# conor722/rust-ray-tracer

Hardware: AMD Instinct MI355X
Metric: Mrays/s (primary) at 1920x1080, Utah teapot (model2.obj) (higher is better)
Workload: dtype f64; 1 GPU; model2.obj 1920x1080, 4 sub-samples/pixel, shadow rays + depth-5 mirror reflection, f64; rays_primary_per_frame=8286720, partition=single launch, octree_nodes=3265, triangles=6334, filter_variant=bundle

## Files before the change

include/rrt.h:

```cpp
#ifndef RRT_H
#define RRT_H
#include <stddef.h>
#include <stdint.h>

#ifdef __cplusplus
extern "C" {
#endif

typedef enum {
    RRT_OK = 0,
    RRT_ERR_INVALID_ARG = -1,
    RRT_ERR_HIP = -2,
    RRT_ERR_OOM = -3,
    RRT_ERR_IO = -4,
    RRT_ERR_PARSE = -5,
    RRT_ERR_DEPTH = -6,
    RRT_ERR_NO_DEVICE = -7,
    RRT_ERR_UNSUPPORTED = -8
} rrt_status;

#define RRT_MAX_OCTREE_DEPTH 40

typedef struct { double x, y, z; } rrt_vec3;

typedef struct { uint32_t kind; uint32_t _pad; double intensity; rrt_vec3 v; } rrt_light;

typedef struct { rrt_vec3 ka, kd, ks; double ns, kr; int32_t tex, bump; } rrt_material;

typedef struct { const uint8_t *rgb; uint32_t width, height; } rrt_texture;

#define RRT_FLAG_NO_CULL 1u
#define RRT_FLAG_LANE_FILTER 2u
#define RRT_FLAG_BUNDLE_FILTER 4u
#define RRT_FLAG_RAY_WALK 8u
#define RRT_FLAG_HOST_SETUP 16u
#define RRT_FLAG_NO_CHAIN_SHORTCUT (1u << 5)

typedef struct {
    double surface_offset;
    uint32_t max_reflection_depth;
    uint32_t flags;
    double vp_w, vp_h, vp_d;
} rrt_options;

typedef struct {
    uint32_t n_tris, n_tris_in_tree;
    uint32_t n_nodes, max_depth;
    uint32_t n_mats, n_tex;
    uint32_t root_own_count, max_own_count;
} rrt_model_info;

// ... 27 lines not shown
void rrt_free(void *p);

typedef struct rrt_raytracer rrt_raytracer;

int rrt_raytracer_create(const rrt_model *m, const rrt_light *lights, uint32_t n_lights, rrt_vec3 origin,
                         const rrt_options *opt, int device, rrt_raytracer **out);
int rrt_raytracer_create_from_arrays(uint32_t n_tris, const double *pos, const double *uv, const double *nrm, const uint32_t *mat,
                                     uint32_t n_mats, const rrt_material *mats, uint32_t n_tex, const rrt_texture *tex, const double *root,
                                     const rrt_light *lights, uint32_t n_lights, rrt_vec3 origin, const rrt_options *opt, int device,
                                     rrt_raytracer **out);
void rrt_raytracer_destroy(rrt_raytracer *rt);

typedef struct { rrt_vec3 eye, right, up, forward; } rrt_camera;
int rrt_raytracer_set_camera(rrt_raytracer *rt, const rrt_camera *cam);
int rrt_raytracer_get_camera(const rrt_raytracer *rt, rrt_camera *out);
int rrt_camera_look_at(rrt_vec3 eye, rrt_vec3 target, rrt_vec3 up_hint, rrt_camera *out);

int rrt_raytracer_set_lights(rrt_raytracer *rt, const rrt_light *lights, uint32_t n_lights);
int rrt_raytracer_get_lights(const rrt_raytracer *rt, rrt_light *out, uint32_t capacity, uint32_t *n_lights);
int rrt_raytracer_set_triangles(rrt_raytracer *rt, uint32_t n_tris, const double *pos, const double *uv, const double *nrm,
                                const uint32_t *mat, const double *root);
int rrt_raytracer_set_triangles_device(rrt_raytracer *rt, uint32_t n_tris, const double *d_pos, const double *d_uv, const double *d_nrm,
                                       const uint32_t *d_mat, const double *root, void *stream);
int rrt_raytracer_release_update_memory(rrt_raytracer *rt);

int rrt_render(rrt_raytracer *rt, uint32_t width, uint32_t height, uint32_t *out_fb);

int rrt_host_buffer_register(void *ptr, size_t bytes);
int rrt_host_buffer_unregister(void *ptr);

// ... 67 lines not shown
```

rust-ray-tracer_amd/__init__.py:

```python
from __future__ import annotations

import ctypes as C
import os
from dataclasses import dataclass
from typing import Iterable, Optional, Sequence

import numpy as np

_HERE = os.path.dirname(os.path.abspath(__file__))
LIB_PATH = os.environ.get("RRT_LIB") or os.path.join(_HERE, "librrt_hip.so")


class RrtError(RuntimeError):
    def __init__(self, status: int, what: str, detail: str):
        super().__init__(f"{what}: {detail or '?'} (status {status})")
        self.status = status
        self.detail = detail


FLAG_NO_CULL, FLAG_LANE_FILTER, FLAG_BUNDLE_FILTER, FLAG_RAY_WALK, FLAG_HOST_SETUP, FLAG_NO_CHAIN_SHORTCUT = 1, 2, 4, 8, 16, 32
BUFFERS = ("nodes", "geom", "attr", "supers", "cboxes", "child_boxes", "tboxes", "suspects", "oct_box", "oct_first_child", "oct_tri_count", "oct_own_off",
           "oct_own_idx", "slot_tri", "slot_pos", "chains")
VARIANT_NAMES = ("lane", "bundle", "ray")

OK, ERR_INVALID_ARG, ERR_HIP, ERR_OOM, ERR_IO, ERR_PARSE, ERR_DEPTH, ERR_NO_DEVICE, ERR_UNSUPPORTED = 0, -1, -2, -3, -4, -5, -6, -7, -8


class Vec3(C.Structure):
    _fields_ = [("x", C.c_double), ("y", C.c_double), ("z", C.c_double)]


class CLight(C.Structure):
    _fields_ = [("kind", C.c_uint32), ("_pad", C.c_uint32), ("intensity", C.c_double), ("v", Vec3)]


# ... 51 lines not shown
    "rrt_model_from_arrays": (C.c_int, [C.c_uint32, _dp, _dp, _dp, _u32p, C.c_uint32, C.POINTER(CMaterial), C.c_uint32, C.POINTER(CTexture), _dp, C.POINTER(_P)]),
    "rrt_model_destroy": (None, [_P]),
    "rrt_model_get_info": (C.c_int, [_P, C.POINTER(CModelInfo)]),
    "rrt_model_get_triangles": (C.c_int, [_P, _dp, _dp, _dp, _u32p]),
    "rrt_model_get_materials": (C.c_int, [_P, C.POINTER(CMaterial)]),
    "rrt_model_get_texture": (C.c_int, [_P, C.c_uint32, C.POINTER(CTexture)]),
    "rrt_model_get_octree": (C.c_int, [_P, _dp, _u32p, _u32p, _u32p, _u32p]),
    "rrt_decode_image_file": (C.c_int, [C.c_char_p, C.POINTER(_u8p), _u32p, _u32p]),
    "rrt_free": (None, [_P]),
    "rrt_raytracer_create": (C.c_int, [_P, C.POINTER(CLight), C.c_uint32, Vec3, C.POINTER(COptions), C.c_int, C.POINTER(_P)]),
    "rrt_raytracer_create_from_arrays": (C.c_int, [C.c_uint32, _dp, _dp, _dp, _u32p, C.c_uint32, C.POINTER(CMaterial), C.c_uint32, C.POINTER(CTexture), _dp,
                                                  C.POINTER(CLight), C.c_uint32, Vec3, C.POINTER(COptions), C.c_int, C.POINTER(_P)]),
    "rrt_raytracer_destroy": (None, [_P]),
    "rrt_raytracer_set_camera": (C.c_int, [_P, C.POINTER(CCamera)]),
    "rrt_raytracer_get_camera": (C.c_int, [_P, C.POINTER(CCamera)]),
    "rrt_camera_look_at": (C.c_int, [Vec3, Vec3, Vec3, C.POINTER(CCamera)]),
    "rrt_raytracer_set_lights": (C.c_int, [_P, C.POINTER(CLight), C.c_uint32]),
    "rrt_raytracer_get_lights": (C.c_int, [_P, C.POINTER(CLight), C.c_uint32, _u32p]),
    "rrt_raytracer_set_triangles": (C.c_int, [_P, C.c_uint32, _dp, _dp, _dp, _u32p, _dp]),
    "rrt_raytracer_set_triangles_device": (C.c_int, [_P, C.c_uint32, _P, _P, _P, _P, _dp, _P]),
    "rrt_raytracer_release_update_memory": (C.c_int, [_P]),
    "rrt_render": (C.c_int, [_P, C.c_uint32, C.c_uint32, _u32p]),
    "rrt_host_buffer_register": (C.c_int, [_P, C.c_size_t]),
    "rrt_host_buffer_unregister": (C.c_int, [_P]),
    "rrt_render_device": (C.c_int, [_P, C.c_uint32, C.c_uint32, _P, _P]),
    "rrt_render_visibility_device": (C.c_int, [_P, C.c_uint32, C.c_uint32, C.POINTER(CRegion), C.POINTER(CVisibility), _P]),
    "rrt_render_visibility": (C.c_int, [_P, C.c_uint32, C.c_uint32, C.POINTER(CRegion), C.POINTER(CVisibility)]),
    "rrt_pick": (C.c_int, [_P, C.c_uint32, C.c_uint32, C.c_uint32, C.c_uint32, C.POINTER(CPickResult)]),
    "rrt_tiles_per_rank": (C.c_uint32, [C.c_uint32, C.c_uint32, C.c_uint32]),
    "rrt_render_tiles_device": (C.c_int, [_P, C.c_uint32, C.c_uint32, C.c_uint32, C.c_uint32, _P, _P]),
# ... 203 lines not shown


def decode_image_file(path: str) -> np.ndarray:
    p = _u8p(); w = C.c_uint32(); h = C.c_uint32()
    _check(lib().rrt_decode_image_file(os.fsencode(path), C.byref(p), C.byref(w), C.byref(h)), f"decode_image_file({path})")
    try:
        return np.ctypeslib.as_array(p, shape=(h.value, w.value, 3)).copy()
    finally:
        lib().rrt_free(p)


class RayTracer:

    def __init__(self, scene_data: SceneData, lights: Iterable[Light], origin: Vector3d = DEFAULT_ORIGIN, device: int = 0,
                 surface_offset: float = 0.0001, max_reflection_depth: int = 5, viewport=(1.0, 1.0, 1.0), no_cull: bool = False,
                 box_filter: Optional[str] = None, host_setup: bool = False, chain_shortcut: bool = True):
        self.scene_data, self.origin, self.device = scene_data, origin, device
        lights = list(lights)
        cl = (CLight * max(1, len(lights)))()
        for i, l in enumerate(lights):
            cl[i] = CLight(l.kind, 0, float(l.intensity), l.v._c())
        flags = (FLAG_NO_CULL if no_cull else 0) | (FLAG_HOST_SETUP if host_setup else 0) | (0 if chain_shortcut else FLAG_NO_CHAIN_SHORTCUT) | {None: 0, "lane": FLAG_LANE_FILTER, "bundle": FLAG_BUNDLE_FILTER, "ray": FLAG_RAY_WALK}[box_filter]
        opt = COptions(surface_offset, max_reflection_depth, flags, *map(float, viewport))
        out = _P()
        _check(lib().rrt_raytracer_create(scene_data._h, cl, len(lights), origin._c(), C.byref(opt), device, C.byref(out)), "rrt_raytracer_create")
        self._h = out

    @classmethod
    def from_arrays(cls, pos, uv, nrm, mat, materials: Sequence[dict], textures: Sequence[np.ndarray], lights: Iterable[Light], origin: Vector3d = DEFAULT_ORIGIN,
                    device: int = 0, root=DEFAULT_ROOT, no_cull: bool = False, box_filter: Optional[str] = None) -> "RayTracer":
        self = cls.__new__(cls)
        self.scene_data, self.origin, self.device = None, origin, device
        lights = list(lights)
        a = _marshal_arrays(pos, uv, nrm, mat, materials, textures, root)
        cl = (CLight * max(1, len(lights)))()
        for i, l in enumerate(lights):
            cl[i] = CLight(l.kind, 0, float(l.intensity), l.v._c())
# ... 43 lines not shown

    def set_camera(self, eye, right=(1.0, 0.0, 0.0), up=(0.0, 1.0, 0.0), forward=(0.0, 0.0, 1.0)) -> None:
        c = CCamera(_vec3(eye), _vec3(right), _vec3(up), _vec3(forward))
        _check(lib().rrt_raytracer_set_camera(self._h, C.byref(c)), "rrt_raytracer_set_camera")

    def look_at(self, eye, target, up=(0.0, 1.0, 0.0)) -> None:
        self.set_camera(**look_at(eye, target, up))

    def reset_camera(self) -> None:
        _check(lib().rrt_raytracer_set_camera(self._h, None), "rrt_raytracer_set_camera")

    def camera(self) -> dict:
        c = CCamera()
        _check(lib().rrt_raytracer_get_camera(self._h, C.byref(c)), "rrt_raytracer_get_camera")
        return _camera_dict(c)

    def set_lights(self, lights: Iterable[Light]) -> None:
        lights = list(lights)
        cl = (CLight * max(1, len(lights)))()
        for i, l in enumerate(lights):
            cl[i] = CLight(l.kind, 0, float(l.intensity), l.v._c())
        _check(lib().rrt_raytracer_set_lights(self._h, cl, len(lights)), "rrt_raytracer_set_lights")

    def lights(self) -> list:
        n = C.c_uint32(0)
        _check(lib().rrt_raytracer_get_lights(self._h, None, 0, C.byref(n)), "rrt_raytracer_get_lights")
        cl = (CLight * max(1, n.value))()
        _check(lib().rrt_raytracer_get_lights(self._h, cl, n.value, C.byref(n)), "rrt_raytracer_get_lights")
        return [Light(l.kind, l.intensity, Vector3d(l.v.x, l.v.y, l.v.z)) for l in cl[:n.value]]

# ... 315 lines not shown
```

rust-ray-tracer_amd/csrc/api_internal.hpp:

```cpp
#pragma once
#include <cstdint>
#include <new>
#include <string>
#include <vector>

#include "device_memory.hpp"
#include "device_scene.hpp"
#include "hip_check.hpp"
#include "model.hpp"
#include "scene_build.hpp"

struct rrt_model { rrt::Model m; };

struct rrt_raytracer {
    int device = 0;
    rrt::DevScene scene{};
    rrt_options opt{};
    rrt::BuiltScene built;
    rrt::DevBuf table_mem; rrt::DevArena tables;
#ifdef RRT_PROFILE
    rrt::DevBuf prof_mem;
#endif
    uint64_t scene_bytes = 0;
    hipEvent_t ev0 = nullptr, ev1 = nullptr;
    rrt_stats stats{};
    bool stats_pending = false;
    bool launched = false;
    int walk = 0;
    int walk_rays = -1;
    bool variant_forced = false;
    rrt::KeptBuf host_fb;
    rrt::KeptBuf vis_buf;
    rrt::KeptBuf tune_buf;
    uint32_t n_chains = 0, n_chain_nodes = 0;
    double upload_ms = 0, hip_init_ms = 0, create_ms = 0;
    bool gpu_setup = false;
    struct Buf { const void* p = nullptr; size_t bytes = 0; } bufs[16];
    hipStream_t own_stream = nullptr;
    uint32_t tuned_w = 0, tuned_h = 0, tuned_world = 0;
    uint32_t size_frames = 0;
    bool size_measured = false;
    rrt_camera cam{};
    rrt_vec3 origin0{};
    rrt::DevBuf guard_mem;
    rrt::Box root{};
    uint64_t built_bytes = 0;
    rrt::BuildMemory update_mem;
};
// ... 48 lines not shown
```

rust-ray-tracer_amd/csrc/device_scene.hpp:

```cpp
#pragma once
#include <cstdint>

namespace rrt {

struct DevNode {
    double lo[3], hi[3];
    double mid[3];
    uint32_t first_child;
    uint32_t sup_begin;
    uint32_t sup_count;
    uint32_t flags;
    uint32_t s0_begin;
    uint32_t leaf_base;
};
static_assert(sizeof(DevNode) == 96, "DevNode must be 96 bytes");

struct DevTriGeom { double v1[3], e1[3], e2[3]; uint32_t pos, _pad; };
static_assert(sizeof(DevTriGeom) == 80, "DevTriGeom must be 80 bytes");
__host__ __device__ inline double edge_canon(double x) {
    uint64_t b; __builtin_memcpy(&b, &x, 8);
    if ((b & 0x7FF0000000000000ull) == 0x7FF0000000000000ull && (b & 0x000FFFFFFFFFFFFFull) != 0ull) b = 0x7FF8000000000000ull;
    __builtin_memcpy(&x, &b, 8);
    return x;
}
// ... 50 lines not shown
    DevLight lights[RRT_MAX_LIGHTS];
#ifdef RRT_PROFILE
    unsigned long long* prof;
#endif
};

struct FrameParams {
    uint32_t width, height;
    double x_scale, y_scale, z_value;
    uint32_t tiles_x, tiles_y;
    uint32_t rank, world;
    uint32_t tiled_output;
    uint32_t xcd_chunk;
    uint32_t tile_begin, tile_end, row_begin, row_end;
    double right[3], up[3], forward[3];
};

struct VisParams {
    FrameParams F;
    uint32_t col_begin, col_end;
    uint32_t tile_x0, tile_y0, tiles_w, _pad;
    uint8_t* hit; double *t, *u, *v; uint32_t* tri; uint32_t* albedo;
};

int launch_render(const DevScene& s, const FrameParams& f, uint32_t* d_out, void* stream, int walk);
int launch_visibility(const DevScene& s, const VisParams& p, void* stream, int walk);
int launch_detile(uint32_t width, uint32_t height, uint32_t world, const uint32_t* d_gathered, uint32_t* d_fb, void* stream);
int launch_ray_colours(const DevScene& s, uint32_t n, const double* d_origins, const double* d_dirs, uint32_t* d_colours, void* stream, int walk);
int launch_intersect(const DevScene& s, uint32_t n, const double* d_origins, const double* d_dirs, const double* d_max_t,
                     uint8_t* d_hit, double* d_t, double* d_u, double* d_v, uint32_t* d_tri, void* stream, int walk);
int launch_occlusion(const DevScene& s, uint32_t n, const double* d_origins, const double* d_dirs, const double* d_max_t, uint8_t* d_occluded, void* stream, int walk);
struct SuspectRecord { uint32_t tri; uint32_t _pad; DevSuspect s; };
int launch_suspects_resident(const DevTriGeom* geom, const DevTriAttr* attr, uint32_t n_list_slots, const double eye[3], double pad,
                             uint32_t* d_count, SuspectRecord* d_out, void* stream);
uint32_t stack_bytes_per_wave(uint32_t levels);
void preload_kernels();

}
```

rust-ray-tracer_amd/csrc/frames.cpp:

```cpp
#include <algorithm>
#include <cstdlib>
#include <cstring>

#include "api_internal.hpp"
#include "staging.hpp"

namespace {

using namespace rrt;

FrameParams frame_params(const rrt_raytracer* rt, uint32_t width, uint32_t height, uint32_t rank, uint32_t world, bool tiled) {
    FrameParams f{};
    f.width = width; f.height = height;
    f.x_scale = rt->opt.vp_w / (double)width;
    f.y_scale = rt->opt.vp_h / (double)height;
    f.z_value = rt->opt.vp_d;
    f.tiles_x = (width + 7) / 8; f.tiles_y = (height + 7) / 8;
    f.rank = rank; f.world = world; f.tiled_output = tiled ? 1u : 0u;
    f.tile_begin = 0; f.tile_end = f.tiles_x * f.tiles_y; f.row_begin = 0; f.row_end = height;
    const rrt_camera& c = rt->cam;
    f.right[0] = c.right.x; f.right[1] = c.right.y; f.right[2] = c.right.z;
    f.up[0] = c.up.x; f.up[1] = c.up.y; f.up[2] = c.up.z;
    f.forward[0] = c.forward.x; f.forward[1] = c.forward.y; f.forward[2] = c.forward.z;
    static const int forced = [] { const char* e = std::getenv("RRT_XCD_CHUNK"); return e ? std::atoi(e) : -1; }();
// ... 80 lines not shown
    if (rt->variant_forced) return rt->walk;
    if (rt->walk_rays >= 0) return rt->walk_rays;
    if (n < kTuneMinRays) return rt->walk;
    return measure_rays(rt, [&](int variant) { return launch(std::min(n, kTuneSample), variant); });
}
int device_rays_variant(const rrt_raytracer* rt) {
    if (rt->variant_forced) return rt->walk;
    return rt->walk_rays >= 0 ? rt->walk_rays : rt->walk;
}
void check_rays(const rrt_raytracer* rt, uint32_t n, const double* origins, const double* dirs, bool outputs_ok) {
    if (!rt) throw Error{RRT_ERR_INVALID_ARG, "null raytracer"};
    if (n && (!origins || !dirs)) throw Error{RRT_ERR_INVALID_ARG, "null ray origins or directions"};
    if (n && !outputs_ok) throw Error{RRT_ERR_INVALID_ARG, "null output: a device form needs one output pointer at least, a host form every one of its outputs"};
}

void launch_frame(rrt_raytracer* rt, uint32_t width, uint32_t height, uint32_t rank, uint32_t world, bool tiled, void* d_out, void* stream) {
    DeviceGuard guard(rt->device);
    const FrameParams f = frame_params(rt, width, height, rank, world, tiled);
    tune_variant(rt, f, static_cast<uint32_t*>(d_out), stream);
    timed_launch(rt, stream, [&] { return launch_render(rt->scene, f, static_cast<uint32_t*>(d_out), stream, rt->walk); });
    record(rt, width, height, world == 1 ? 4 * traced_pixels(width, height) : 0, rt->walk);
}

int visibility_variant(const rrt_raytracer* rt, uint32_t width, uint32_t height) {
    if (rt->variant_forced) return rt->walk;
    if (rt->tuned_w == width && rt->tuned_h == height && rt->tuned_world == 1u) return rt->walk;
    return first_frame_variant(rt, width, height);
}

constexpr int kPlanes = 6;
constexpr size_t kPlaneElem[kPlanes] = {1, 8, 8, 8, 4, 4};

rrt_region check_visibility(const rrt_raytracer* rt, uint32_t width, uint32_t height, const rrt_region* region, const rrt_visibility* planes) {
// ... 137 lines not shown
        visibility_to_host(rt, width, height, r, *planes);
        return RRT_OK;
    });
}

int rrt_pick(rrt_raytracer* rt, uint32_t width, uint32_t height, uint32_t px, uint32_t py, rrt_pick_result* out) {
    return guarded([&]() -> int {
        check_frame(rt, width, height);
        if (!out) throw Error{RRT_ERR_INVALID_ARG, "null result"};
        if (px >= width || py >= height) throw Error{RRT_ERR_INVALID_ARG, "pixel outside the frame"};
        *out = pick_pixel(rt, width, height, px, py);
        return RRT_OK;
    });
}

int rrt_detile_device(rrt_raytracer* rt, uint32_t width, uint32_t height, uint32_t world, const void* d_gathered, void* d_fb, void* stream) {
    return guarded([&]() -> int {
        check_frame(rt, width, height);
        if (!d_gathered || !d_fb || world == 0) throw Error{RRT_ERR_INVALID_ARG, "bad argument"};
        DeviceGuard guard(rt->device);
        HIP_TRY((hipError_t)launch_detile(width, height, world, static_cast<const uint32_t*>(d_gathered), static_cast<uint32_t*>(d_fb), stream));
        return RRT_OK;
    });
}

int rrt_host_buffer_register(void* ptr, size_t bytes) {
    return guarded([&]() -> int {
        if (!ptr || !bytes) throw Error{RRT_ERR_INVALID_ARG, "null buffer"};
        HIP_TRY(hipHostRegister(ptr, bytes, hipHostRegisterDefault));
        return RRT_OK;
// ... 19 lines not shown
        staged_download(out_fb, d_fb, bytes, rt->own_stream);
        HIP_TRY(hipStreamSynchronize(rt->own_stream));
        return RRT_OK;
    });
}

int rrt_render_progressive(rrt_raytracer* rt, uint32_t width, uint32_t height, uint32_t* out_fb, uint32_t chunk_rows, rrt_update_fn on_update, void* user) {
    return guarded([&]() -> int {
        check_frame(rt, width, height);
        if (!out_fb) throw Error{RRT_ERR_INVALID_ARG, "null framebuffer"};
        if (chunk_rows == 0) chunk_rows = 50;
        DeviceGuard guard(rt->device);
        const size_t bytes = sizeof(uint32_t) * (size_t)width * height;
        uint32_t* d_fb = static_cast<uint32_t*>(rt->host_fb.at_least(bytes));
        FrameParams f = frame_params(rt, width, height, 0, 1, false);
        tune_variant(rt, f, d_fb, nullptr);
        HIP_TRY(hipMemsetAsync(d_fb, 0, bytes, nullptr));
        std::memset(out_fb, 0, bytes);
        const int64_t H = height, half = H / 2;
        timed_launch(rt, nullptr, [&] {
            for (int64_t cs = -half; cs < half; cs += chunk_rows) {
                const int64_t ce = std::min<int64_t>(cs + chunk_rows, half);
                const int64_t r_lo = H - (ce - 1 + half), r_hi = std::min<int64_t>(H - (cs + half), H - 1);
                if (r_lo <= r_hi) {
                    f.row_begin = (uint32_t)r_lo; f.row_end = (uint32_t)r_hi + 1;
                    f.tile_begin = (f.row_begin / 8) * f.tiles_x; f.tile_end = ((f.row_end + 7) / 8) * f.tiles_x;
                    HIP_TRY((hipError_t)launch_render(rt->scene, f, d_fb, nullptr, rt->walk));
                    HIP_TRY(hipMemcpy(out_fb + (size_t)f.row_begin * width, d_fb + (size_t)f.row_begin * width,
                                      sizeof(uint32_t) * (size_t)width * (f.row_end - f.row_begin), hipMemcpyDeviceToHost));
                }
// ... 123 lines not shown
```

rust-ray-tracer_amd/csrc/raytracer.cpp:

```cpp
#include <atomic>
#include <chrono>
#include <cstdio>
#include <cstdlib>
#include <cstring>
#include <functional>
#include <memory>

#include "api_internal.hpp"
#include "parallel.hpp"
#include "staging.hpp"

namespace {

using namespace rrt;

enum { kBufNodes = 0, kBufGeom, kBufAttr, kBufSupers, kBufCboxes, kBufChildBoxes, kBufTboxes, kBufSuspects, kBufOctBox, kBufOctFirstChild, kBufOctTriCount, kBufOctOwnOff, kBufOctOwnIdx, kBufSlotTri, kBufSlotPos, kBufChains, kBufCount };

void alloc_tables(rrt_raytracer* rt, const SceneTables& T) {
    size_t need = (size_t)1 << 16;
    for (auto& t : T.tex) need += (size_t)3 * t.width * t.height + 256;
    need += T.n_mats * sizeof(DevMaterial) + T.tex.size() * sizeof(DevTexture) + 1024;
    rt->table_mem = dev_alloc(need);
    rt->tables.base = static_cast<char*>(rt->table_mem.h); rt->tables.cap = need;
}
// ... 49 lines not shown
        {kBufSlotTri, G.slot_tri, (size_t)G.n_slots_total * 4}, {kBufSlotPos, G.slot_pos, (size_t)G.n_slots_total * 4},
        {kBufChains, G.chains, (size_t)G.n_chains * sizeof(DevChain)}};
    for (const auto& k : kept) { rt->bufs[k.id].p = k.p; rt->bufs[k.id].bytes = k.p ? k.bytes : 0; }
    S.cull_enabled = (o.flags & RRT_FLAG_NO_CULL) ? 0u : 1u;
    S.cull_half_over_limit = S.cull_limit > 0.0f ? 0.5f / S.cull_limit : 0.0f;
    S.inner_shrink = (S.cull_enabled && G.all_inside_root) ? (float)(2.0 * G.pad) : 0.0f;
    rt->n_chains = G.n_chains; rt->n_chain_nodes = G.n_chain_nodes;
    if (!(S.inner_shrink > 0.0f)) { rt->n_chains = 0; rt->n_chain_nodes = 0; }
    S.chains = (rt->n_chains && !(o.flags & RRT_FLAG_NO_CHAIN_SHORTCUT)) ? G.chains : nullptr;
    S.n_suspects = G.n_suspects;
    S.stack_levels = G.max_depth > 1 ? G.max_depth - 1 : 1;
    const uint64_t bytes = (uint64_t)G.n_nodes * sizeof(DevNode) + (uint64_t)G.n_slots_total * (sizeof(DevTriGeom) + sizeof(DevTriAttr))
                         + ((uint64_t)G.n_sup_records + n_cboxes + n_child_boxes + n_tboxes) * 32;
    rt->scene_bytes += bytes - rt->built_bytes;
    rt->built_bytes = bytes;
}

void check_lights(const rrt_light* lights, uint32_t n_lights) {
    if (n_lights && !lights) throw Error{RRT_ERR_INVALID_ARG, "null light list"};
    if (n_lights > RRT_MAX_LIGHTS) throw Error{RRT_ERR_INVALID_ARG, "too many lights (max 16)"};
    for (uint32_t i = 0; i < n_lights; i++) if (lights[i].kind > 2) throw Error{RRT_ERR_INVALID_ARG, "bad light kind"};
}

void store_lights(rrt_raytracer* rt, const rrt_light* lights, uint32_t n_lights) {
    DevScene& S = rt->scene;
    S.n_lights = n_lights;
    for (uint32_t i = 0; i < n_lights; i++) {
        S.lights[i].kind = lights[i].kind; S.lights[i]._pad = 0; S.lights[i].intensity = lights[i].intensity;
        S.lights[i].v[0] = lights[i].v.x; S.lights[i].v[1] = lights[i].v.y; S.lights[i].v[2] = lights[i].v.z;
    }
// ... 208 lines not shown
```

rust-ray-tracer_amd/csrc/render.hip:

```cpp
#include <hip/hip_runtime.h>

#include <cmath>
#include <type_traits>

#include "device_scene.hpp"

#ifndef RRT_TU
#define RRT_TU 0
#endif
#define RRT_TU_FRAME (RRT_TU == 0 || RRT_TU == 1)
#define RRT_TU_LANE (RRT_TU == 0 || RRT_TU == 3)
#define RRT_TU_RAYS (RRT_TU == 0 || RRT_TU == 2)

namespace rrt {
namespace {

#define RRT_CONSTANT __attribute__((address_space(4)))
constexpr double kEps = 2.220446049250313e-16;
constexpr uint32_t kNone = 0xFFFFFFFFu;
constexpr double kInf = __builtin_huge_val();

struct V3 { double x, y, z; };
__device__ __forceinline__ V3 mk(double x, double y, double z) { V3 r; r.x = x; r.y = y; r.z = z; return r; }
__device__ __forceinline__ V3 ld3(const double* p) { return mk(p[0], p[1], p[2]); }
// ... 1234 lines not shown
    uint32_t blk = blockIdx.x;
    if (F.xcd_chunk) {
        const uint32_t C = F.xcd_chunk, full = (gridDim.x / (8u * C)) * (8u * C);
        if (blk < full) { const uint32_t xcd = blk & 7u, i = blk >> 3; blk = ((i / C) * 8u + xcd) * C + (i % C); }
    }
    const uint32_t local_tile = blk >> 2, quad = blk & 3u;
    const uint32_t pix = lane >> 2, sub = lane & 3u;
    const uint32_t tile = F.tile_begin + local_tile * F.world + F.rank;
    const bool tile_ok = tile < F.tile_end;
    const uint32_t tx = tile_ok ? tile % F.tiles_x : 0, ty = tile_ok ? tile / F.tiles_x : 0;
    const uint32_t px = tx * 8 + (quad & 1u) * 4 + (pix & 3u);
    const uint32_t py = ty * 8 + (quad >> 1) * 4 + (pix >> 2);
    const int32_t W = (int32_t)F.width, H = (int32_t)F.height;
    const bool in_fb = tile_ok && (int32_t)px < W && py >= F.row_begin && py < F.row_end;
    const bool traced = in_fb && (int32_t)px < 2 * (W / 2) && (int32_t)py >= H - 2 * (H / 2) + 1;
    const int32_t x = (int32_t)px - W / 2;
    const int32_t y = (H - H / 2) - (int32_t)py;
    const double xd = (sub & 1u) ? ((double)x + 0.5) : (double)x;
    const double yd = (sub & 2u) ? ((double)y + 0.5) : (double)y;
    const double sa = xd * F.x_scale, sb = yd * F.y_scale, sc = F.z_value;
    const V3 dir = mk((F.right[0] * sa + F.up[0] * sb) + F.forward[0] * sc,
                      (F.right[1] * sa + F.up[1] * sb) + F.forward[1] * sc,
                      (F.right[2] * sa + F.up[2] * sb) + F.forward[2] * sc);
#ifdef RRT_PROFILE
    Prof prof{}; prof.last = __builtin_amdgcn_s_memtime();
    const unsigned long long wave_rt0 = __builtin_amdgcn_s_memrealtime(); (void)wave_rt0;
#endif
    const uint32_t c = trace_colour<kWalk, kGroups, true>(PROF_ARG S, stk, traced, ld3(S.origin), dir);
#if defined(RRT_PROFILE) && defined(RRT_PROF_WAVETIME)
    {
        constexpr unsigned long long kRealtimeTicksPerUs = 100ull;
        const unsigned long long ticks = __builtin_amdgcn_s_memrealtime() - wave_rt0;
        const uint32_t us = (uint32_t)(ticks / kRealtimeTicksPerUs);
        const uint32_t bucket = us < 2u ? 0u : (uint32_t)(31 - __builtin_clz(us));
        if (lane == 0) { atomicAdd(S.prof + (bucket < 15u ? bucket : 15u), 1ull); atomicMax(S.prof + 16, ticks); }
    }
#elif defined(RRT_PROFILE)
    PROF_T(4);
    for (int i = 0; i < 16; i++) if (prof.c[i]) atomicAdd(S.prof + i, prof.c[i]);
    if (lane == 0) { for (int i = 0; i < 8; i++) if (prof.t[i]) atomicAdd(S.prof + 16 + i, prof.t[i]); }
    for (int i = 0; i < 4; i++) if (prof.b[i]) atomicAdd(S.prof + 24 + i, prof.b[i]);
#endif
    uint32_t r = (c >> 16) & 255u, g = (c >> 8) & 255u, b = c & 255u;
// ... 323 lines not shown
```

rust-ray-tracer_amd/csrc/scene_build.hip:

```cpp
#include <cfloat>
#include <cmath>
#include <cstdio>
#include <cstdlib>
#include <cstring>

#include <hip/hip_runtime.h>
#include <rocprim/rocprim.hpp>

#include <algorithm>
#include <chrono>
#include <memory>
#include <string>
#include <vector>

#include "parallel.hpp"
#include "scene_build.hpp"
#include "staging.hpp"

namespace rrt {
namespace {

constexpr uint32_t kNone = 0xFFFFFFFFu;
constexpr int kBlock = 256;
constexpr uint32_t kClusterTris = 8, kSuperTris = 64, kGroupSupers = 8, kGroupThreshold = 24;
// ... 539 lines not shown
    const double v1[3] = {t.v1.x, t.v1.y, t.v1.z};
    const double e1[3] = {t.v2.x - t.v1.x, t.v2.y - t.v1.y, t.v2.z - t.v1.z}, e2[3] = {t.v3.x - t.v1.x, t.v3.y - t.v1.y, t.v3.z - t.v1.z};
    DevSuspect q;
    if (suspect_of(v1, e1, e2, ox, oy, oz, pad, q)) suspect_append(i, q, count, out);
}
__global__ void __launch_bounds__(kBlock) k_suspects_resident(const DevTriGeom* __restrict__ geom, const DevTriAttr* __restrict__ attr, uint32_t n_list_slots,
                                                              double ox, double oy, double oz, double pad, uint32_t* count, SuspectRecord* out) {
    const uint32_t s = blockIdx.x * kBlock + threadIdx.x;
    if (s >= n_list_slots) return;
    const DevTriGeom& g = geom[s];
    const double v1[3] = {g.v1[0], g.v1[1], g.v1[2]}, e1[3] = {g.e1[0], g.e1[1], g.e1[2]}, e2[3] = {g.e2[0], g.e2[1], g.e2[2]};
    DevSuspect q;
    if (suspect_of(v1, e1, e2, ox, oy, oz, pad, q)) suspect_append(attr[s].orig, q, count, out);
}

__global__ void __launch_bounds__(kBlock) k_pack_triangles(const double* __restrict__ pos, const double* __restrict__ uv, const double* __restrict__ nrm, const uint32_t* __restrict__ mat, uint32_t n, Triangle* __restrict__ out) {
    const uint32_t i = blockIdx.x * kBlock + threadIdx.x;
    if (i >= n) return;
    auto rd = [](const double* p) { Vec3 v; v.x = p[0]; v.y = p[1]; v.z = p[2]; return v; };
    Triangle t;
    t.v1 = rd(pos + 9 * (size_t)i); t.v2 = rd(pos + 9 * (size_t)i + 3); t.v3 = rd(pos + 9 * (size_t)i + 6);
    t.t1 = rd(uv + 9 * (size_t)i);  t.t2 = rd(uv + 9 * (size_t)i + 3);  t.t3 = rd(uv + 9 * (size_t)i + 6);
    t.n1 = rd(nrm + 9 * (size_t)i); t.n2 = rd(nrm + 9 * (size_t)i + 3); t.n3 = rd(nrm + 9 * (size_t)i + 6);
    t.mat = mat[i]; t._pad = 0;
    out[i] = t;
}
__global__ void __launch_bounds__(kBlock) k_count_bad_materials(const uint32_t* __restrict__ mat, uint32_t n, uint32_t n_mats, uint32_t* count) {
    __shared__ uint32_t block_count;
    if (threadIdx.x == 0) block_count = 0u;
    __syncthreads();
// ... 282 lines not shown
    if (e != hipSuccess) return (int)e;
    if (n == 0) return 0;
    hipLaunchKernelGGL(k_count_bad_materials, dim3(std::min(grid_for(n), 1024u)), dim3(kBlock), 0, st, d_mat, n, n_mats, d_count);
    return (int)hipGetLastError();
}

int launch_suspects_resident(const DevTriGeom* geom, const DevTriAttr* attr, uint32_t n_list_slots, const double eye[3], double pad, uint32_t* d_count, SuspectRecord* d_out, void* stream) {
    hipStream_t st = (hipStream_t)stream;
    hipError_t e = hipMemsetAsync(d_count, 0, sizeof(uint32_t), st);
    if (e != hipSuccess) return (int)e;
    if (n_list_slots == 0) return 0;
    hipLaunchKernelGGL(k_suspects_resident, dim3(grid_for(n_list_slots)), dim3(kBlock), 0, st, geom, attr, n_list_slots, eye[0], eye[1], eye[2], pad, d_count, d_out);
    return (int)hipGetLastError();
}

}
```

Baseline: 10450 Mrays/s.

## Skip tracing screen quads that no triangle cluster box can project onto

A new kernel projects every leaf cluster bounding box through the camera with conservative error bounds. It sets bits in a per-resolution mask of 4x4-pixel quads, and any degenerate or unsafe case falls back to a full mask. The render kernel reads this mask and, for uncovered quads, writes the background colour directly without building a ray or walking the hierarchy. The mask is cached per resolution and keyed on camera, viewport and scene epoch, so it is rebuilt only when those change. The cost is an extra small launch whenever the view changes, plus correctness risk if the conservative bounds are ever too tight.

```diff
diff --git a/include/rrt.h b/include/rrt.h
--- a/include/rrt.h
+++ b/include/rrt.h
@@ -35,6 +35,7 @@
 #define RRT_FLAG_RAY_WALK 8u
 #define RRT_FLAG_HOST_SETUP 16u
 #define RRT_FLAG_NO_CHAIN_SHORTCUT (1u << 5)
+#define RRT_FLAG_NO_COVERAGE (1u << 6)
 
 typedef struct {
     double surface_offset;
@@ -92,6 +93,7 @@
 typedef struct { rrt_vec3 eye, right, up, forward; } rrt_camera;
 int rrt_raytracer_set_camera(rrt_raytracer *rt, const rrt_camera *cam);
 int rrt_raytracer_get_camera(const rrt_raytracer *rt, rrt_camera *out);
+int rrt_raytracer_get_coverage(rrt_raytracer *rt, uint32_t width, uint32_t height, uint32_t *words, uint32_t capacity, uint32_t *n_words, uint32_t *flags);
 int rrt_camera_look_at(rrt_vec3 eye, rrt_vec3 target, rrt_vec3 up_hint, rrt_camera *out);
 
 int rrt_raytracer_set_lights(rrt_raytracer *rt, const rrt_light *lights, uint32_t n_lights);
diff --git a/rust-ray-tracer_amd/__init__.py b/rust-ray-tracer_amd/__init__.py
--- a/rust-ray-tracer_amd/__init__.py
+++ b/rust-ray-tracer_amd/__init__.py
@@ -18,7 +18,7 @@
         self.detail = detail
 
 
-FLAG_NO_CULL, FLAG_LANE_FILTER, FLAG_BUNDLE_FILTER, FLAG_RAY_WALK, FLAG_HOST_SETUP, FLAG_NO_CHAIN_SHORTCUT = 1, 2, 4, 8, 16, 32
+FLAG_NO_CULL, FLAG_LANE_FILTER, FLAG_BUNDLE_FILTER, FLAG_RAY_WALK, FLAG_HOST_SETUP, FLAG_NO_CHAIN_SHORTCUT, FLAG_NO_COVERAGE = 1, 2, 4, 8, 16, 32, 64
 BUFFERS = ("nodes", "geom", "attr", "supers", "cboxes", "child_boxes", "tboxes", "suspects", "oct_box", "oct_first_child", "oct_tri_count", "oct_own_off",
            "oct_own_idx", "slot_tri", "slot_pos", "chains")
 VARIANT_NAMES = ("lane", "bundle", "ray")
@@ -100,6 +100,7 @@
     "rrt_raytracer_destroy": (None, [_P]),
     "rrt_raytracer_set_camera": (C.c_int, [_P, C.POINTER(CCamera)]),
     "rrt_raytracer_get_camera": (C.c_int, [_P, C.POINTER(CCamera)]),
+    "rrt_raytracer_get_coverage": (C.c_int, [_P, C.c_uint32, C.c_uint32, _u32p, C.c_uint32, _u32p, _u32p]),
     "rrt_camera_look_at": (C.c_int, [Vec3, Vec3, Vec3, C.POINTER(CCamera)]),
     "rrt_raytracer_set_lights": (C.c_int, [_P, C.POINTER(CLight), C.c_uint32]),
     "rrt_raytracer_get_lights": (C.c_int, [_P, C.POINTER(CLight), C.c_uint32, _u32p]),
@@ -333,13 +334,13 @@
 
     def __init__(self, scene_data: SceneData, lights: Iterable[Light], origin: Vector3d = DEFAULT_ORIGIN, device: int = 0,
                  surface_offset: float = 0.0001, max_reflection_depth: int = 5, viewport=(1.0, 1.0, 1.0), no_cull: bool = False,
-                 box_filter: Optional[str] = None, host_setup: bool = False, chain_shortcut: bool = True):
+                 box_filter: Optional[str] = None, host_setup: bool = False, chain_shortcut: bool = True, coverage: bool = True):
         self.scene_data, self.origin, self.device = scene_data, origin, device
         lights = list(lights)
         cl = (CLight * max(1, len(lights)))()
         for i, l in enumerate(lights):
             cl[i] = CLight(l.kind, 0, float(l.intensity), l.v._c())
-        flags = (FLAG_NO_CULL if no_cull else 0) | (FLAG_HOST_SETUP if host_setup else 0) | (0 if chain_shortcut else FLAG_NO_CHAIN_SHORTCUT) | {None: 0, "lane": FLAG_LANE_FILTER, "bundle": FLAG_BUNDLE_FILTER, "ray": FLAG_RAY_WALK}[box_filter]
+        flags = (FLAG_NO_CULL if no_cull else 0) | (FLAG_HOST_SETUP if host_setup else 0) | (0 if chain_shortcut else FLAG_NO_CHAIN_SHORTCUT) | (0 if coverage else FLAG_NO_COVERAGE) | {None: 0, "lane": FLAG_LANE_FILTER, "bundle": FLAG_BUNDLE_FILTER, "ray": FLAG_RAY_WALK}[box_filter]
         opt = COptions(surface_offset, max_reflection_depth, flags, *map(float, viewport))
         out = _P()
         _check(lib().rrt_raytracer_create(scene_data._h, cl, len(lights), origin._c(), C.byref(opt), device, C.byref(out)), "rrt_raytracer_create")
@@ -413,6 +414,15 @@
         c = CCamera()
         _check(lib().rrt_raytracer_get_camera(self._h, C.byref(c)), "rrt_raytracer_get_camera")
         return _camera_dict(c)
+
+    def coverage(self, w: int, h: int) -> dict:
+        n = C.c_uint32(0); fl = C.c_uint32(0)
+        _check(lib().rrt_raytracer_get_coverage(self._h, w, h, None, 0, C.byref(n), C.byref(fl)), "rrt_raytracer_get_coverage")
+        words = np.full(n.value, 0xFFFFFFFF, np.uint32)
+        _check(lib().rrt_raytracer_get_coverage(self._h, w, h, words.ctypes.data_as(_u32p), n.value, None, C.byref(fl)), "rrt_raytracer_get_coverage")
+        qx, qy = 2 * ((w + 7) // 8), 2 * ((h + 7) // 8)
+        bits = np.unpackbits(words.view(np.uint8), bitorder="little")[:qx * qy].reshape(qy, qx).astype(bool)
+        return {"bits": bits, "in_use": bool(fl.value & 1), "full": bool(fl.value & 2)}
 
     def set_lights(self, lights: Iterable[Light]) -> None:
         lights = list(lights)
diff --git a/rust-ray-tracer_amd/csrc/api_internal.hpp b/rust-ray-tracer_amd/csrc/api_internal.hpp
--- a/rust-ray-tracer_amd/csrc/api_internal.hpp
+++ b/rust-ray-tracer_amd/csrc/api_internal.hpp
@@ -11,6 +11,20 @@
 #include "scene_build.hpp"
 
 struct rrt_model { rrt::Model m; };
+
+namespace rrt {
+struct CoverageMask {
+    uint32_t width = 0, height = 0, n_words = 0;
+    struct Key { uint64_t epoch; double v[15]; } key{};
+    bool valid = false;
+    bool in_use = false;
+    KeptBuf buf;
+    HipOwned<hipEvent_t, hipEventDestroy> built;
+    hipStream_t built_on = nullptr;
+    bool settled = false;
+};
+constexpr size_t kMaxCoverageSizes = 8;
+}
 
 struct rrt_raytracer {
     int device = 0;
@@ -32,6 +46,8 @@
     rrt::KeptBuf host_fb;
     rrt::KeptBuf vis_buf;
     rrt::KeptBuf tune_buf;
+    std::vector<rrt::CoverageMask> coverage;
+    uint64_t scene_epoch = 0;
     uint32_t n_chains = 0, n_chain_nodes = 0;
     double upload_ms = 0, hip_init_ms = 0, create_ms = 0;
     bool gpu_setup = false;
diff --git a/rust-ray-tracer_amd/csrc/device_scene.hpp b/rust-ray-tracer_amd/csrc/device_scene.hpp
--- a/rust-ray-tracer_amd/csrc/device_scene.hpp
+++ b/rust-ray-tracer_amd/csrc/device_scene.hpp
@@ -88,6 +88,7 @@
     uint32_t xcd_chunk;
     uint32_t tile_begin, tile_end, row_begin, row_end;
     double right[3], up[3], forward[3];
+    const uint32_t* coverage;
 };
 
 struct VisParams {
@@ -107,6 +108,13 @@
 struct SuspectRecord { uint32_t tri; uint32_t _pad; DevSuspect s; };
 int launch_suspects_resident(const DevTriGeom* geom, const DevTriAttr* attr, uint32_t n_list_slots, const double eye[3], double pad,
                              uint32_t* d_count, SuspectRecord* d_out, void* stream);
+struct CoverageView {
+    double eye[3];
+    double inv[9];
+    double z_value, x_scale, y_scale;
+    uint32_t width, height, quads_x, quads_y;
+};
+int launch_coverage(const DevClusterBox* tboxes, uint32_t n_list_slots, const CoverageView& v, uint32_t* d_mask, uint32_t n_words, void* stream);
 uint32_t stack_bytes_per_wave(uint32_t levels);
 void preload_kernels();
 
diff --git a/rust-ray-tracer_amd/csrc/frames.cpp b/rust-ray-tracer_amd/csrc/frames.cpp
--- a/rust-ray-tracer_amd/csrc/frames.cpp
+++ b/rust-ray-tracer_amd/csrc/frames.cpp
@@ -1,4 +1,5 @@
 #include <algorithm>
+#include <cmath>
 #include <cstdlib>
 #include <cstring>
 
@@ -118,9 +119,81 @@
     if (n && !outputs_ok) throw Error{RRT_ERR_INVALID_ARG, "null output: a device form needs one output pointer at least, a host form every one of its outputs"};
 }
 
+bool coverage_view(const rrt_raytracer* rt, uint32_t width, uint32_t height, CoverageView& v) {
+    static const bool env_on = [] { const char* e = std::getenv("RRT_COVERAGE"); return !(e && std::atoi(e) == 0); }();
+    const DevScene& S = rt->scene;
+    if (!env_on || (rt->opt.flags & (RRT_FLAG_NO_CULL | RRT_FLAG_NO_COVERAGE)) || !S.cull_enabled || !(rt->built.pad > 0) || S.n_suspects > 0 || S.n_slots >= 50000u) return false;
+    const FrameParams f = frame_params(rt, width, height, 0, 1, false);
+    if (!(f.z_value != 0.0) || !std::isfinite(f.z_value) || !std::isfinite(f.x_scale) || !std::isfinite(f.y_scale)) return false;
+    const double* r = f.right; const double* u = f.up; const double* w = f.forward;
+    const double cof[9] = {u[1] * w[2] - u[2] * w[1], u[2] * w[0] - u[0] * w[2], u[0] * w[1] - u[1] * w[0],
+                           w[1] * r[2] - w[2] * r[1], w[2] * r[0] - w[0] * r[2], w[0] * r[1] - w[1] * r[0],
+                           r[1] * u[2] - r[2] * u[1], r[2] * u[0] - r[0] * u[2], r[0] * u[1] - r[1] * u[0]};
+    const double det = r[0] * cof[0] + r[1] * cof[1] + r[2] * cof[2];
+    if (!(det != 0.0) || !std::isfinite(det)) return false;
+    double norm_m = 0, norm_inv = 0;
+    for (int i = 0; i < 3; i++) {
+        double row = 0;
+        for (int k = 0; k < 3; k++) { v.inv[3 * i + k] = cof[3 * i + k] / det; row += std::fabs(v.inv[3 * i + k]); }
+        norm_inv = std::max(norm_inv, row);
+        norm_m = std::max(norm_m, std::fabs(r[i]) + std::fabs(u[i]) + std::fabs(w[i]));
+    }
+    if (!std::isfinite(norm_inv) || !(norm_m * norm_inv <= 0x1p16)) return false;
+    const double limit = S.cull_limit;
+    if (!std::isfinite(limit)) return false;
+    const double ha = std::fabs(f.x_scale) * (width / 2 + 1.0), hb = std::fabs(f.y_scale) * (height / 2 + 1.0), hc = std::fabs(f.z_value);
+    for (int k = 0; k < 3; k++) {
+        if (!(std::fabs(S.origin[k]) <= limit)) return false;
+        if (!(std::fabs(r[k]) * ha + std::fabs(u[k]) * hb + std::fabs(w[k]) * hc <= limit)) return false;
+        v.eye[k] = S.origin[k];
+    }
+    v.z_value = f.z_value; v.x_scale = f.x_scale; v.y_scale = f.y_scale;
+    v.width = width; v.height = height; v.quads_x = 2 * f.tiles_x; v.quads_y = 2 * f.tiles_y;
+    return true;
+}
+
+CoverageMask* ensure_coverage(rrt_raytracer* rt, uint32_t width, uint32_t height, void* stream) {
+    CoverageMask* m = nullptr;
+    for (CoverageMask& c : rt->coverage) if (c.width == width && c.height == height) m = &c;
+    if (!m) {
+        if (rt->coverage.size() >= kMaxCoverageSizes) return nullptr;
+        rt->coverage.emplace_back();
+        m = &rt->coverage.back(); m->width = width; m->height = height;
+    }
+    CoverageMask::Key key{};
+    key.epoch = rt->scene_epoch;
+    const rrt_camera& c = rt->cam;
+    const double vals[15] = {rt->scene.origin[0], rt->scene.origin[1], rt->scene.origin[2], c.right.x, c.right.y, c.right.z, c.up.x, c.up.y, c.up.z,
+                             c.forward.x, c.forward.y, c.forward.z, rt->opt.vp_w, rt->opt.vp_h, rt->opt.vp_d};
+    std::memcpy(key.v, vals, sizeof vals);
+    if (!(m->valid && std::memcmp(&m->key, &key, sizeof key) == 0)) {
+        m->valid = false;
+        CoverageView v{};
+        m->in_use = coverage_view(rt, width, height, v);
+        if (m->in_use) {
+            m->n_words = (v.quads_x * v.quads_y + 31u) / 32u;
+            uint32_t* d_mask = static_cast<uint32_t*>(m->buf.at_least(sizeof(uint32_t) * ((size_t)m->n_words + 1)));
+            if (!m->built.h) HIP_TRY(hipEventCreateWithFlags(&m->built.h, hipEventDisableTiming));
+            HIP_TRY((hipError_t)launch_coverage(rt->scene.tboxes, rt->built.n_list_slots, v, d_mask, m->n_words, stream));
+            HIP_TRY(hipEventRecord(m->built.h, (hipStream_t)stream));
+            m->built_on = (hipStream_t)stream; m->settled = false;
+        }
+        m->key = key; m->valid = true;
+    } else if (m->in_use && !m->settled) {
+        if (hipEventQuery(m->built.h) == hipSuccess) m->settled = true;
+        else if ((hipStream_t)stream != m->built_on) HIP_TRY(hipStreamWaitEvent((hipStream_t)stream, m->built.h, 0));
+    }
+    return m->in_use ? m : nullptr;
+}
+const uint32_t* coverage_words(rrt_raytracer* rt, uint32_t width, uint32_t height, void* stream) {
+    const CoverageMask* m = ensure_coverage(rt, width, height, stream);
+    return m ? static_cast<const uint32_t*>(m->buf.mem.h) : nullptr;
+}
+
 void launch_frame(rrt_raytracer* rt, uint32_t width, uint32_t height, uint32_t rank, uint32_t world, bool tiled, void* d_out, void* stream) {
     DeviceGuard guard(rt->device);
-    const FrameParams f = frame_params(rt, width, height, rank, world, tiled);
+    FrameParams f = frame_params(rt, width, height, rank, world, tiled);
+    f.coverage = coverage_words(rt, width, height, stream);
     tune_variant(rt, f, static_cast<uint32_t*>(d_out), stream);
     timed_launch(rt, stream, [&] { return launch_render(rt->scene, f, static_cast<uint32_t*>(d_out), stream, rt->walk); });
     record(rt, width, height, world == 1 ? 4 * traced_pixels(width, height) : 0, rt->walk);
@@ -288,6 +361,30 @@
     });
 }
 
+int rrt_raytracer_get_coverage(rrt_raytracer* rt, uint32_t width, uint32_t height, uint32_t* words, uint32_t capacity, uint32_t* n_words, uint32_t* flags) {
+    return guarded([&]() -> int {
+        check_frame(rt, width, height);
+        if (capacity && !words) throw Error{RRT_ERR_INVALID_ARG, "null words with a non-zero capacity"};
+        DeviceGuard guard(rt->device);
+        const uint32_t n = (4u * ((width + 7) / 8) * ((height + 7) / 8) + 31u) / 32u;
+        if (n_words) *n_words = n;
+        if (!rt->own_stream) rt->own_stream = (hipStream_t)setup_stream();
+        const CoverageMask* m = ensure_coverage(rt, width, height, rt->own_stream);
+        uint32_t fl = 0;
+        if (m) {
+            const uint32_t* d_mask = static_cast<const uint32_t*>(m->buf.mem.h);
+            uint32_t full = 0;
+            const uint32_t k = std::min(capacity, m->n_words);
+            if (k) HIP_TRY(hipMemcpyAsync(words, d_mask, sizeof(uint32_t) * (size_t)k, hipMemcpyDeviceToHost, rt->own_stream));
+            HIP_TRY(hipMemcpyAsync(&full, d_mask + m->n_words, sizeof full, hipMemcpyDeviceToHost, rt->own_stream));
+            HIP_TRY(hipStreamSynchronize(rt->own_stream));
+            fl = 1u | (full ? 2u : 0u);
+        }
+        if (flags) *flags = fl;
+        return RRT_OK;
+    });
+}
+
 int rrt_detile_device(rrt_raytracer* rt, uint32_t width, uint32_t height, uint32_t world, const void* d_gathered, void* d_fb, void* stream) {
     return guarded([&]() -> int {
         check_frame(rt, width, height);
@@ -337,6 +434,7 @@
         const size_t bytes = sizeof(uint32_t) * (size_t)width * height;
         uint32_t* d_fb = static_cast<uint32_t*>(rt->host_fb.at_least(bytes));
         FrameParams f = frame_params(rt, width, height, 0, 1, false);
+        f.coverage = coverage_words(rt, width, height, nullptr);
         tune_variant(rt, f, d_fb, nullptr);
         HIP_TRY(hipMemsetAsync(d_fb, 0, bytes, nullptr));
         std::memset(out_fb, 0, bytes);
diff --git a/rust-ray-tracer_amd/csrc/raytracer.cpp b/rust-ray-tracer_amd/csrc/raytracer.cpp
--- a/rust-ray-tracer_amd/csrc/raytracer.cpp
+++ b/rust-ray-tracer_amd/csrc/raytracer.cpp
@@ -87,6 +87,7 @@
                          + ((uint64_t)G.n_sup_records + n_cboxes + n_child_boxes + n_tboxes) * 32;
     rt->scene_bytes += bytes - rt->built_bytes;
     rt->built_bytes = bytes;
+    rt->scene_epoch++;
 }
 
 void check_lights(const rrt_light* lights, uint32_t n_lights) {
diff --git a/rust-ray-tracer_amd/csrc/render.hip b/rust-ray-tracer_amd/csrc/render.hip
--- a/rust-ray-tracer_amd/csrc/render.hip
+++ b/rust-ray-tracer_amd/csrc/render.hip
@@ -1272,19 +1272,27 @@
     const int32_t W = (int32_t)F.width, H = (int32_t)F.height;
     const bool in_fb = tile_ok && (int32_t)px < W && py >= F.row_begin && py < F.row_end;
     const bool traced = in_fb && (int32_t)px < 2 * (W / 2) && (int32_t)py >= H - 2 * (H / 2) + 1;
-    const int32_t x = (int32_t)px - W / 2;
-    const int32_t y = (H - H / 2) - (int32_t)py;
-    const double xd = (sub & 1u) ? ((double)x + 0.5) : (double)x;
-    const double yd = (sub & 2u) ? ((double)y + 0.5) : (double)y;
-    const double sa = xd * F.x_scale, sb = yd * F.y_scale, sc = F.z_value;
-    const V3 dir = mk((F.right[0] * sa + F.up[0] * sb) + F.forward[0] * sc,
-                      (F.right[1] * sa + F.up[1] * sb) + F.forward[1] * sc,
-                      (F.right[2] * sa + F.up[2] * sb) + F.forward[2] * sc);
+    bool covered = true;
+    if (F.coverage) {
+        const uint32_t bit = (2u * ty + (quad >> 1)) * (2u * F.tiles_x) + 2u * tx + (quad & 1u);
+        covered = ((((const RRT_CONSTANT uint32_t*)F.coverage)[bit >> 5] >> (bit & 31u)) & 1u) != 0u;
+    }
 #ifdef RRT_PROFILE
     Prof prof{}; prof.last = __builtin_amdgcn_s_memtime();
     const unsigned long long wave_rt0 = __builtin_amdgcn_s_memrealtime(); (void)wave_rt0;
 #endif
-    const uint32_t c = trace_colour<kWalk, kGroups, true>(PROF_ARG S, stk, traced, ld3(S.origin), dir);
+    uint32_t c = 0x00FFFFFFu;
+    if (covered) {
+        const int32_t x = (int32_t)px - W / 2;
+        const int32_t y = (H - H / 2) - (int32_t)py;
+        const double xd = (sub & 1u) ? ((double)x + 0.5) : (double)x;
+        const double yd = (sub & 2u) ? ((double)y + 0.5) : (double)y;
+        const double sa = xd * F.x_scale, sb = yd * F.y_scale, sc = F.z_value;
+        const V3 dir = mk((F.right[0] * sa + F.up[0] * sb) + F.forward[0] * sc,
+                          (F.right[1] * sa + F.up[1] * sb) + F.forward[1] * sc,
+                          (F.right[2] * sa + F.up[2] * sb) + F.forward[2] * sc);
+        c = trace_colour<kWalk, kGroups, true>(PROF_ARG S, stk, traced, ld3(S.origin), dir);
+    }
 #if defined(RRT_PROFILE) && defined(RRT_PROF_WAVETIME)
     {
         constexpr unsigned long long kRealtimeTicksPerUs = 100ull;
diff --git a/rust-ray-tracer_amd/csrc/scene_build.hip b/rust-ray-tracer_amd/csrc/scene_build.hip
--- a/rust-ray-tracer_amd/csrc/scene_build.hip
+++ b/rust-ray-tracer_amd/csrc/scene_build.hip
@@ -577,6 +577,63 @@
     if (suspect_of(v1, e1, e2, ox, oy, oz, pad, q)) suspect_append(attr[s].orig, q, count, out);
 }
 
+__global__ void __launch_bounds__(kBlock) k_coverage(const DevClusterBox* __restrict__ tboxes, uint32_t n_list_slots, CoverageView V, uint32_t* words, uint32_t* full) {
+    const uint32_t s = blockIdx.x * kBlock + threadIdx.x;
+    if (s >= n_list_slots) return;
+    const DevClusterBox B = tboxes[s];
+    if (B.h[0] < 0.0f || B.h[1] < 0.0f || B.h[2] < 0.0f) return;
+    if (B.h[0] >= FLT_MAX || B.h[1] >= FLT_MAX || B.h[2] >= FLT_MAX) { *full = 1u; return; }
+    constexpr double kEps8 = 8.0 * 0x1p-53;
+    double ea = 0, eb = 0, ew = 0;
+    for (int j = 0; j < 3; j++) {
+        const double P = fabs((double)B.c[j]) + (double)B.h[j] + fabs(V.eye[j]);
+        ea += fabs(V.inv[j]) * P; eb += fabs(V.inv[3 + j]) * P; ew += fabs(V.inv[6 + j]) * P;
+    }
+    ea *= kEps8; eb *= kEps8; ew *= kEps8 / fabs(V.z_value);
+    double wmin = INFINITY, wmax = -INFINITY, a[8], b[8], w[8];
+    for (int k = 0; k < 8; k++) {
+        const double p[3] = {((double)B.c[0] + ((k & 1) ? (double)B.h[0] : -(double)B.h[0])) - V.eye[0],
+                             ((double)B.c[1] + ((k & 2) ? (double)B.h[1] : -(double)B.h[1])) - V.eye[1],
+                             ((double)B.c[2] + ((k & 4) ? (double)B.h[2] : -(double)B.h[2])) - V.eye[2]};
+        a[k] = V.inv[0] * p[0] + V.inv[1] * p[1] + V.inv[2] * p[2];
+        b[k] = V.inv[3] * p[0] + V.inv[4] * p[1] + V.inv[5] * p[2];
+        w[k] = (V.inv[6] * p[0] + V.inv[7] * p[1] + V.inv[8] * p[2]) / V.z_value;
+        if (!isfinite(a[k]) || !isfinite(b[k]) || !isfinite(w[k])) { *full = 1u; return; }
+        wmin = fmin(wmin, w[k]); wmax = fmax(wmax, w[k]);
+    }
+    if (!isfinite(ea + eb + ew)) { *full = 1u; return; }
+    if (wmax < -ew) return;
+    if (!(wmin > 1024.0 * ew)) { *full = 1u; return; }
+    double x0 = INFINITY, x1 = -INFINITY, y0 = INFINITY, y1 = -INFINITY;
+    for (int k = 0; k < 8; k++) {
+        const double dx = w[k] * V.x_scale, dy = w[k] * V.y_scale;
+        const double x = a[k] / dx + (double)(V.width / 2u);
+        const double y = (double)(V.height - V.height / 2u) - b[k] / dy;
+        const double ex = 1.01 * (ea + fabs(a[k]) * (ew / w[k])) / fabs(dx) + kEps8 * fabs(x);
+        const double ey = 1.01 * (eb + fabs(b[k]) * (ew / w[k])) / fabs(dy) + kEps8 * fabs(y);
+        if (!isfinite(x) || !isfinite(y) || !(ex <= 0.5) || !(ey <= 0.5)) { *full = 1u; return; }
+        x0 = fmin(x0, x); x1 = fmax(x1, x); y0 = fmin(y0, y); y1 = fmax(y1, y);
+    }
+    constexpr double kGrow = 1.5;
+    const double W = (double)V.width, H = (double)V.height;
+    x0 = floor(x0 - kGrow); x1 = ceil(x1 + kGrow); y0 = floor(y0 - kGrow); y1 = ceil(y1 + kGrow);
+    if (x1 < 0.0 || y1 < 0.0 || x0 > W - 1.0 || y0 > H - 1.0) return;
+    const uint32_t qx0 = (uint32_t)fmax(x0, 0.0) >> 2, qx1 = min((uint32_t)fmin(x1, W - 1.0) >> 2, V.quads_x - 1u);
+    const uint32_t qy0 = (uint32_t)fmax(y0, 0.0) >> 2, qy1 = min((uint32_t)fmin(y1, H - 1.0) >> 2, V.quads_y - 1u);
+    for (uint32_t qy = qy0; qy <= qy1; qy++) {
+        const uint32_t first = qy * V.quads_x + qx0, last = qy * V.quads_x + qx1;
+        for (uint32_t wd = first >> 5; wd <= (last >> 5); wd++) {
+            const uint32_t lo = wd == (first >> 5) ? (first & 31u) : 0u, hi = wd == (last >> 5) ? (last & 31u) : 31u;
+            const uint32_t bits = (0xFFFFFFFFu >> (31u - hi)) & (0xFFFFFFFFu << lo);
+            if ((__atomic_load_n(words + wd, __ATOMIC_RELAXED) & bits) != bits) atomicOr(words + wd, bits);
+        }
+    }
+}
+__global__ void __launch_bounds__(kBlock) k_coverage_full(uint32_t* words, uint32_t n_words, const uint32_t* full) {
+    const uint32_t i = blockIdx.x * kBlock + threadIdx.x;
+    if (i < n_words && *full) words[i] = 0xFFFFFFFFu;
+}
+
 __global__ void __launch_bounds__(kBlock) k_pack_triangles(const double* __restrict__ pos, const double* __restrict__ uv, const double* __restrict__ nrm, const uint32_t* __restrict__ mat, uint32_t n, Triangle* __restrict__ out) {
     const uint32_t i = blockIdx.x * kBlock + threadIdx.x;
     if (i >= n) return;
@@ -889,4 +946,14 @@
     return (int)hipGetLastError();
 }
 
-}
+int launch_coverage(const DevClusterBox* tboxes, uint32_t n_list_slots, const CoverageView& v, uint32_t* d_mask, uint32_t n_words, void* stream) {
+    hipStream_t st = (hipStream_t)stream;
+    hipError_t e = hipMemsetAsync(d_mask, 0, sizeof(uint32_t) * ((size_t)n_words + 1), st);
+    if (e != hipSuccess) return (int)e;
+    if (n_list_slots == 0) return 0;
+    hipLaunchKernelGGL(k_coverage, dim3(grid_for(n_list_slots)), dim3(kBlock), 0, st, tboxes, n_list_slots, v, d_mask, d_mask + n_words);
+    hipLaunchKernelGGL(k_coverage_full, dim3(grid_for(n_words)), dim3(kBlock), 0, st, d_mask, n_words, d_mask + n_words);
+    return (int)hipGetLastError();
+}
+
+}
```

Result: faster. 11050 Mrays/s (median of 6 runs) (+5.7%).
